# lmxyy/sige

Measured on AMD Instinct MI355X. Metric: DDPM-256 U-Net sparse (SIGE) forwards/s, higher is better.
Workload: dtype f32; 1 GPU; DDPM 256x256 church U-Net (ch128, mult 1-1-2-2-4-4, 113.7M params, random init), 1.2% square edit, one edited image per GPU, hipGraph replay, NHWC activations, in-place scatter ...; batch_per_gpu=1, resolution=256, parallelism=dp1

## Files before the change

### include/sige_hip.h

```cpp
#ifndef SIGE_HIP_H
#define SIGE_HIP_H

#include <stddef.h>
#include <stdint.h>

#ifdef __cplusplus
extern "C" {
#endif

#define SIGE_HIP_VERSION 309

enum {
    SIGE_HIP_OK = 0,
    SIGE_HIP_EINVAL = -1,
    SIGE_HIP_EUNSUPPORTED = -2,
    SIGE_HIP_ELAUNCH = -3,
    SIGE_HIP_ENODEVICE = -4
};

enum { SIGE_HIP_ACT_IDENTITY = 0, SIGE_HIP_ACT_SWISH = 1,
       SIGE_HIP_ACT_RELU = 2, SIGE_HIP_ACT_LEAKY = 3 , SIGE_HIP_ACT_TANH = 4 };

enum {
    SIGE_HIP_TUNE_CONV_TILE_MT = 0,
// ... 343 lines not shown
int sige_hip_conv3x3_small_cin_tiles_nhwc_f32(const float *x, int64_t strideB, int64_t strideC, int64_t strideH, int64_t strideW,
                                              int B, int Cin, int H, int W,
                                              const float *weight, const float *bias, int Cout,
                                              const int32_t *active_indices, int N, int bH, int bW,
                                              float *out, void *stream);

size_t sige_hip_group_norm_affine_workspace(int B, int C, int H, int W, int groups);
int sige_hip_group_norm_affine_f32(const float *x, int B, int C, int H, int W, int groups, float eps,
                                   const float *gamma, const float *beta, float *workspace,
                                   float *scale, float *shift, void *stream);

size_t sige_hip_group_norm_affine_nhwc_workspace(int B, int C, int H, int W, int groups);
int sige_hip_group_norm_affine_nhwc_f32(const float *x, int B, int C, int H, int W, int groups, float eps,
                                        const float *gamma, const float *beta, float *workspace,
                                        float *scale, float *shift, void *stream);

int sige_hip_group_norm_affine_nhwc_bias_f32(const float *x, int B, int C, int H, int W, int groups, float eps,
                                             const float *gamma, const float *beta, const float *channel_bias,
                                             float *workspace, float *scale, float *shift, void *stream);

int sige_hip_group_norm_affine_from_stats_f32(const float *stats1, int tiles1, int C1, int count1,
                                              const float *stats2, int tiles2, int C2, int count2,
                                              int B, int groups, float eps, const float *gamma, const float *beta,
                                              const float *channel_bias, float *scale, float *shift, void *stream);

int sige_hip_channel_stats_tiles(int H, int W);
int sige_hip_channel_stats_nhwc_f32(const float *x, int B, int C, int H, int W, float *stats, void *stream);

size_t sige_hip_attention_workspace(int B, int C, int HW);
int sige_hip_attention_f32(const float *qkv, int B, int C, int HW, float scale, float *workspace,
                           float *out, void *stream);
int sige_hip_attention_nhwc_f32(const float *qkv, int B, int C, int HW, float scale, float *workspace,
                                float *out, void *stream);
size_t sige_hip_attention_fused_workspace(int B, int C, int HW);
int sige_hip_attention_fused_nhwc_f32(const float *qkv, int B, int C, int HW, float scale, float *workspace,
                                      float *out, void *stream);

size_t sige_hip_block_conv_packed_size_f16x3(int Cout, int Cin, int kH, int kW, int R, int S,
                                            int strideH, int strideW, int groups);
int sige_hip_block_conv_pack_f16x3(const float *w, int Cout, int Cin, int kH, int kW,
                                  float *packed, void *stream);
int sige_hip_block_conv_nhwc_f16x3(const float *x, int T, int Cin, int R, int S,
                                  const float *packed, const float *bias, int Cout, int kH, int kW,
                                  int strideH, int strideW, float *out, void *stream);
int sige_hip_block_conv_nhwc_keyed(int compute, const float *x, const int32_t *count_key, int B, int N, int Cin, int R, int S,
                                   const float *packed, const float *bias, int Cout, int kH, int kW,
                                   int strideH, int strideW, float *out, void *stream);
int sige_hip_gather_conv_nhwc_f16x3(const float *x, const float *x2, int B, int C1, int C2, int H, int W,
                                   int bH, int bW, const int32_t *active_indices, int N,
                                   const float *scale, int scaleB, int scaleC,
                                   const float *shift, int shiftB, int shiftC,
                                   int activation,
                                   const float *packed, const float *bias, int Cout, int kH, int kW,
                                   int strideH, int strideW,
                                   int to_full, int offsetH, int offsetW, const float *residual, int Ho, int Wo,
                                   float *workspace, size_t workspace_floats,
                                   const float *out_scale, const float *out_shift, int out_activation,
                                   int upsample2x,
                                   float *twin0, const float *twin0_scale, const float *twin0_shift,
                                   float *twin1, const float *twin1_scale, const float *twin1_shift,
                                   float *out, void *stream);
int sige_hip_scatter_gather_conv_nhwc_f16x3(const float *x, const float *y, int B, int Cin, int H, int W,
                                           int Rx, int Sx, int bH, int bW,
                                           const int32_t *active_indices, int N, const int32_t *scatter_map,
                                           const float *scale, int scaleB, int scaleC,
                                           const float *shift, int shiftB, int shiftC,
// ... 106 lines not shown
```

### sige_amd/build.py

```python
import os
import subprocess
import sys

PKG = os.path.dirname(os.path.abspath(__file__))
REPO = os.path.dirname(PKG)
CSRC = os.path.join(PKG, "csrc")
LIB_DIR = os.path.join(PKG, "lib")
LIB = os.path.join(LIB_DIR, "libsige_hip.so")
SOURCES = ["api.hip", "plan.hip", "gather.hip", "scatter.hip", "reduce_mask.hip", "mask_pipeline.hip", "block_conv.hip", "conv_k3s1.hip", "conv_k1.hip",
           "conv_k3s2.hip", "conv_k3s1_nhwc.hip", "conv_k1_nhwc.hip", "conv_k3s2_nhwc.hip", "conv_k3s1_nhwc_w8.hip", "conv_k1_nhwc_w8.hip", "conv_k3s1_nhwc_h.hip", "conv_k1_nhwc_h.hip", "conv_k3s1_nhwc_x.hip", "conv_k1_nhwc_x.hip", "conv_k3s1_nhwc_c16.hip", "conv_k3s1_nhwc_h_c16.hip", "conv_k3s1_nhwc_x_c16.hip", "conv_pair_nhwc_x_t4.hip", "conv_pair_nhwc_x_f4.hip",
           "conv_pair_nhwc_t4.hip", "conv_pair_nhwc_t8.hip", "conv_pair_nhwc_f4.hip", "conv_pair_nhwc_f8.hip", "conv_pair_nhwc_h_t4.hip", "conv_pair_nhwc_h_f4.hip", "conv_wide.hip", "conv_wide_k3_p8.hip", "conv_wide_k3_f32.hip", "conv_wide_k1_p8.hip", "conv_wide_pair_f32.hip", "conv_wide_pair_x3.hip", "conv_wide_pair_f16.hip", "group_norm.hip", "attention.hip", "attention_fused.hip", "attention_tokens.hip", "nhwc_ops.hip", "conv_out.hip", "conv_in.hip", "spade_ops.hip", "conv_tile3.hip", "conv_tile3_f32.hip", "token_ops.hip", "conv_tile3_f16.hip"]
FLAGS = ["--offload-arch=gfx950", "-O3", "-std=c++17", "-fPIC", "-ffp-contract=off", "-Wno-unused-result"]


def source_hash() -> str:
    import hashlib

    h = hashlib.sha256(" ".join(FLAGS).encode())
    for f in sorted(os.listdir(CSRC)):
        if f.endswith((".hip", ".hpp", ".h")):
            h.update(f.encode())
            h.update(open(os.path.join(CSRC, f), "rb").read())
    h.update(open(os.path.join(REPO, "include", "sige_hip.h"), "rb").read())
    return h.hexdigest()[:16]
# ... 19 lines not shown
        return True
    t = os.path.getmtime(obj)
    return any(os.path.getmtime(d) > t for d in [src, *headers])


TUNING_UNITS = ("api.hip", "block_conv.hip", "gather.hip", "conv_wide.hip", "attention_tokens.hip", "conv_out.hip", "conv_tile3.hip")
TUNING_LIB = os.path.join(LIB_DIR, "libsige_hip_tuning.so")


def _compile_cmd(src: str, obj: str, defs=()):
    return [_hipcc(), *FLAGS, "-DSIGE_TU_ID=%d" % SOURCES.index(src), *defs, "-I" + os.path.join(REPO, "include"), "-I" + CSRC, "-c",
            os.path.join(CSRC, src), "-o", obj]


def _headers():
    headers = [os.path.join(CSRC, f) for f in os.listdir(CSRC) if f.endswith((".hpp", ".h"))]
    headers.append(os.path.join(REPO, "include", "sige_hip.h"))
    return headers


def _headers_of(src: str, headers):
    return (headers if src.startswith("conv_wide") else [h for h in headers if not h.endswith("conv_wide.hpp")] if src.startswith(("conv_k", "conv_pair", "conv_tile3", "block_conv"))
            else [h for h in headers if not h.endswith(("conv_mfma.hpp", "conv_wide.hpp", "conv_tile3.hpp"))])


def _run_all(procs):
    for cmd, p in procs:
        if p.wait() != 0:
            raise RuntimeError("hipcc failed: " + " ".join(cmd))


def build_tuning(force: bool = False, verbose: bool = True) -> str:
    build(force=force, verbose=verbose)
    tdir = os.path.join(LIB_DIR, "tuning")
    os.makedirs(tdir, exist_ok=True)
    headers = _headers()
    objs, procs = [], []
    for src in SOURCES:
        if src in TUNING_UNITS:
            obj = os.path.join(tdir, src.replace(".hip", ".o"))
            if force or _stale(obj, os.path.join(CSRC, src), _headers_of(src, headers)):
                cmd = _compile_cmd(src, obj, ["-DSIGE_HIP_TUNING"])
                if verbose:
                    print(" ".join(cmd), flush=True)
                procs.append((cmd, subprocess.Popen(cmd)))
        else:
            obj = os.path.join(LIB_DIR, src.replace(".hip", ".o"))
        objs.append(obj)
    _run_all(procs)
    if procs or not os.path.isfile(TUNING_LIB) or os.path.getmtime(TUNING_LIB) < os.path.getmtime(LIB):
        subprocess.check_call([_hipcc(), "--offload-arch=gfx950", "-shared", "-fPIC", *objs, "-o", TUNING_LIB])
    return TUNING_LIB


def build_probe(verbose: bool = True) -> str:
    build_tuning(verbose=verbose)
    tag = os.environ.get("SIGE_PROBE_TAG", "")
    only = os.environ.get("SIGE_PROBE_ONLY", "").split()
    pdir = os.path.join(LIB_DIR, "probe" + tag)
    os.makedirs(pdir, exist_ok=True)
    objs, procs = [], []
    wide = bool(os.environ.get("SIGE_PROBE_WIDE"))
    for src in SOURCES:
        if (src.startswith("conv_wide") if wide else
                src.startswith(("conv_k", "conv_pair", "conv_tile3", "block_conv")) and (not only or src in only or src.startswith("block_conv"))):
            obj = os.path.join(pdir, src.replace(".hip", ".o"))
# ... 51 lines not shown
```

### sige_amd/csrc/nhwc_ops.hip

```cpp
#include "common.hpp"

namespace sige {

constexpr int kT = 256;

__device__ __forceinline__ float4 ld4(const float *p) { return *reinterpret_cast<const float4 *>(p); }
__device__ __forceinline__ void st4(float *p, float4 v) { *reinterpret_cast<float4 *>(p) = v; }
__device__ __forceinline__ void st4_out(float *p, float4 v) { store_out4(p, v); }
typedef _Float16 h16x4 __attribute__((ext_vector_type(4)));
__device__ __forceinline__ float4 ld4(const _Float16 *p) {
    const h16x4 h = *reinterpret_cast<const h16x4 *>(p);
    return make_float4((float)h[0], (float)h[1], (float)h[2], (float)h[3]);
}
__device__ __forceinline__ void st4(_Float16 *p, float4 v) {
    const h16x4 h = {(_Float16)v.x, (_Float16)v.y, (_Float16)v.z, (_Float16)v.w};
    *reinterpret_cast<h16x4 *>(p) = h;
}

template <int ACT>
__device__ __forceinline__ float4 affine_act4(float4 z, const float *scale, const float *shift, int so, int c) {
    if (scale) { const float4 s = ld4(scale + so + c); z.x = s.x * z.x; z.y = s.y * z.y; z.z = s.z * z.z; z.w = s.w * z.w; }
    if (shift) { const float4 s = ld4(shift + so + c); z.x = s.x + z.x; z.y = s.y + z.y; z.z = s.z + z.z; z.w = s.w + z.w; }
    z.x = activate<ACT>(z.x); z.y = activate<ACT>(z.y); z.z = activate<ACT>(z.z); z.w = activate<ACT>(z.w);
    return z;
// ... 196 lines not shown
    const int b = blockIdx.z;
    const int i0 = blockIdx.y * 16, j0 = blockIdx.x * 16;
    const int tid = threadIdx.x, wave = tid >> 6, lane = tid & 63;
    const int kq = lane >> 4, n = lane & 15;
    const int C3 = 3 * C, cw = C / 4;
    const float *qa = qkv + ((size_t)b * HW + i0 + n) * C3 + wave * cw + kq * 4;
    const float *kb = qkv + ((size_t)b * HW + j0 + n) * C3 + C + wave * cw + kq * 4;
    f32x4 acc0 = {0.f, 0.f, 0.f, 0.f}, acc1 = {0.f, 0.f, 0.f, 0.f};
    for (int s0 = 0; s0 < cw; s0 += 128) {
        float4 a4[8], b4[8];
#pragma unroll
        for (int u = 0; u < 8; ++u) {
            const int s = s0 + 16 * u;
            const bool ok = s < cw;
            a4[u] = ok ? ld4(qa + s) : make_float4(0.f, 0.f, 0.f, 0.f);
            b4[u] = ok ? ld4(kb + s) : make_float4(0.f, 0.f, 0.f, 0.f);
        }
#pragma unroll
        for (int u = 0; u < 8; ++u) {
            acc0 = __builtin_amdgcn_mfma_f32_16x16x4f32(a4[u].x, b4[u].x, acc0, 0, 0, 0);
            acc1 = __builtin_amdgcn_mfma_f32_16x16x4f32(a4[u].y, b4[u].y, acc1, 0, 0, 0);
            acc0 = __builtin_amdgcn_mfma_f32_16x16x4f32(a4[u].z, b4[u].z, acc0, 0, 0, 0);
            acc1 = __builtin_amdgcn_mfma_f32_16x16x4f32(a4[u].w, b4[u].w, acc1, 0, 0, 0);
        }
    }
#pragma unroll
    for (int r = 0; r < 4; ++r) red[wave][4 * kq + r][n] = acc0[r] + acc1[r];
    __syncthreads();
    const int qi = tid >> 4, kj = tid & 15;
    const float v = (red[0][qi][kj] + red[1][qi][kj]) + (red[2][qi][kj] + red[3][qi][kj]);
    S[((size_t)b * HW + i0 + qi) * HW + j0 + kj] = v * scale;
}

__global__ __launch_bounds__(kT) void attn_apply_nhwc_kernel(const float *__restrict__ qkv, const float *__restrict__ S,
                                                            int C, int HW, float *__restrict__ out) {
    extern __shared__ __attribute__((aligned(16))) float P[];
    const int PS = HW + 4;
    const int b = blockIdx.z;
    const int i0 = blockIdx.y * 16, c0 = blockIdx.x * 64;
    const int tid = threadIdx.x, wave = tid >> 6, lane = tid & 63;
    const int kq = lane >> 4, n = lane & 15;
    const int c = c0 + wave * 16 + n;
    const bool cok = c < C;
    const size_t rs = (size_t)3 * C;
    const __amdgpu_buffer_rsrc_t r_v = __builtin_amdgcn_make_buffer_rsrc(
        const_cast<float *>(qkv + (size_t)b * HW * 3 * C + 2 * C), 0,
        (unsigned)min((size_t)0x7fffffff, ((size_t)HW * 3 * C - 2 * C) * sizeof(float)), 0x00020000);
    const int v_lane = ((cok ? c : 0) + kq * (int)rs) * (int)sizeof(float);
    const int v_step = 4 * (int)rs * (int)sizeof(float);
    float bv[64];
    auto load_values = [&](int j0) {
        const int nk = min(256, HW - j0) / 4;
#pragma unroll
        for (int u = 0; u < 64; ++u)
            bv[u] = __builtin_bit_cast(float, __builtin_amdgcn_raw_buffer_load_b32(r_v, v_lane, (j0 / 4 + min(u, nk - 1)) * v_step, 0));
    };
    {
        const int row = tid >> 4, l16 = tid & 15;
        const float *srow = S + ((size_t)b * HW + i0 + row) * HW;
        if (HW <= 256) {
            float4 t[4];
#pragma unroll
            for (int u = 0; u < 4; ++u) {
                const int j = l16 * 4 + 64 * u;
                const float4 q4 = ld4(srow + min(j, HW - 4));
                t[u] = j < HW ? q4 : make_float4(-INFINITY, -INFINITY, -INFINITY, -INFINITY);
            }
            load_values(0);
            float m = -INFINITY;
#pragma unroll
            for (int u = 0; u < 4; ++u) m = fmaxf(fmaxf(m, fmaxf(t[u].x, t[u].y)), fmaxf(t[u].z, t[u].w));
            m = row16_max(m);
            float sum = 0.f;
#pragma unroll
            for (int u = 0; u < 4; ++u) {
                if (l16 * 4 + 64 * u < HW) {
                    t[u].x = expf(t[u].x - m); t[u].y = expf(t[u].y - m); t[u].z = expf(t[u].z - m); t[u].w = expf(t[u].w - m);
                    sum += (t[u].x + t[u].y) + (t[u].z + t[u].w);
                }
            }
            sum = row16_sum(sum);
            const float inv = 1.0f / sum;
#pragma unroll
            for (int u = 0; u < 4; ++u) {
                const int j = l16 * 4 + 64 * u;
                if (j < HW) {
                    t[u].x *= inv; t[u].y *= inv; t[u].z *= inv; t[u].w *= inv;
                    st4(P + row * PS + j, t[u]);
                }
            }
        } else {
            load_values(0);
            float m = -INFINITY;
            for (int j = l16 * 4; j < HW; j += 64) {
                const float4 t = ld4(srow + j);
                st4(P + row * PS + j, t);
                m = fmaxf(fmaxf(m, fmaxf(t.x, t.y)), fmaxf(t.z, t.w));
            }
#pragma unroll
            for (int o = 8; o > 0; o >>= 1) m = fmaxf(m, __shfl_xor(m, o, 16));
            float sum = 0.f;
            for (int j = l16 * 4; j < HW; j += 64) {
                float4 t = ld4(P + row * PS + j);
                t.x = expf(t.x - m); t.y = expf(t.y - m); t.z = expf(t.z - m); t.w = expf(t.w - m);
                sum += (t.x + t.y) + (t.z + t.w);
                st4(P + row * PS + j, t);
            }
#pragma unroll
            for (int o = 8; o > 0; o >>= 1) sum += __shfl_xor(sum, o, 16);
            const float inv = 1.0f / sum;
            for (int j = l16 * 4; j < HW; j += 64) {
                float4 t = ld4(P + row * PS + j);
                t.x *= inv; t.y *= inv; t.z *= inv; t.w *= inv;
                st4(P + row * PS + j, t);
            }
        }
    }
    __syncthreads();
    const float *pa = P + n * PS + kq;
    f32x4 acc0 = {0.f, 0.f, 0.f, 0.f}, acc1 = {0.f, 0.f, 0.f, 0.f};
    for (int j0 = 0; j0 < HW; j0 += 256) {
        const int nk = min(256, HW - j0) / 4;
        if (j0 > 0) load_values(j0);
#pragma unroll
        for (int u = 0; u < 64; ++u) {
            const float av = pa[j0 + 4 * min(u, nk - 1)];
            const float bb = u < nk ? bv[u] : 0.f;
            if (u & 1) acc1 = __builtin_amdgcn_mfma_f32_16x16x4f32(av, bb, acc1, 0, 0, 0);
            else acc0 = __builtin_amdgcn_mfma_f32_16x16x4f32(av, bb, acc0, 0, 0, 0);
        }
    }
    if (cok) {
#pragma unroll
        for (int r = 0; r < 4; ++r) out[((size_t)b * HW + i0 + 4 * kq + r) * C + c] = acc0[r] + acc1[r];
    }
}

}

using namespace sige;

static bool al16(const void *p) { return (reinterpret_cast<uintptr_t>(p) & 15) == 0; }

static bool affine_shape(const float *scale, int sB, int sC, const float *shift, int tB, int tC, int B, int C, int *aff_sb) {
    *aff_sb = 0;
    for (int k = 0; k < 2; ++k) {
        const float *p = k ? shift : scale;
        const int pb = k ? tB : sB, pc = k ? tC : sC;
        if (!p) continue;
        if (!((pb == 1 || pb == B) && pc == C) || !al16(p)) return false;
        if (pb > 1) *aff_sb = C;
    }
    if (scale && shift && sB != tB) return false;
    return true;
}

template <typename XT>
static int gather_nhwc_impl(const XT *x, int B, int C, int H, int W, int bH, int bW,
                            const int32_t *active_indices, int N,
                            const float *scale, int scaleB, int scaleC,
                            const float *shift, int shiftB, int shiftC,
                            int activation, float *out, void *stream) {
    if (B < 0 || C <= 0 || H <= 0 || W <= 0 || bH <= 0 || bW <= 0 || N < 0) return SIGE_HIP_EINVAL;
    if (activation != SIGE_HIP_ACT_IDENTITY && activation != SIGE_HIP_ACT_SWISH) return SIGE_HIP_EUNSUPPORTED;
    const int hp_shift = stacked_shift(H);
    if (hp_shift < 0 || (hp_shift && B != 1)) return SIGE_HIP_EUNSUPPORTED;
    if ((long)B * N == 0) return SIGE_HIP_OK;
// ... 248 lines not shown
template <typename ST, typename DT>
__global__ __launch_bounds__(kT) void convert4_kernel(const ST *__restrict__ src, DT *__restrict__ dst, size_t n4) {
    for (size_t u = (size_t)blockIdx.x * kT + threadIdx.x; u < n4; u += (size_t)gridDim.x * kT) st4(dst + u * 4, ld4(src + u * 4));
}

extern "C" int sige_hip_convert_f16_f32(const void *src, float *dst, size_t n, void *stream) {
    SIGE_PLAN_HOOK(sige_hip_convert_f16_f32, src, dst, n, stream);
    if (!src || !dst) return SIGE_HIP_EINVAL;
    if (n == 0) return SIGE_HIP_OK;
    if (n % 4 || (reinterpret_cast<uintptr_t>(src) & 7) || !al16(dst)) return SIGE_HIP_EUNSUPPORTED;
    convert4_kernel<_Float16, float><<<grid_for((long)(n / 4)), kT, 0, as_stream(stream)>>>(static_cast<const _Float16 *>(src), dst, n / 4);
    return launch_status();
}

extern "C" int sige_hip_convert_f32_f16(const float *src, void *dst, size_t n, void *stream) {
    SIGE_PLAN_HOOK(sige_hip_convert_f32_f16, src, dst, n, stream);
    if (!src || !dst) return SIGE_HIP_EINVAL;
    if (n == 0) return SIGE_HIP_OK;
    if (n % 4 || (reinterpret_cast<uintptr_t>(dst) & 7) || !al16(src)) return SIGE_HIP_EUNSUPPORTED;
    convert4_kernel<float, _Float16><<<grid_for((long)(n / 4)), kT, 0, as_stream(stream)>>>(src, static_cast<_Float16 *>(dst), n / 4);
    return launch_status();
}

extern "C" int sige_hip_attention_nhwc_f32(const float *qkv, int B, int C, int HW, float scale, float *workspace,
                                           float *out, void *stream) {
    SIGE_PLAN_HOOK(sige_hip_attention_nhwc_f32, qkv, B, C, HW, scale, workspace, out, stream);
    if (B <= 0 || C <= 0 || HW <= 0) return SIGE_HIP_EINVAL;
    if (!qkv || !workspace || !out) return SIGE_HIP_EINVAL;
    if (HW % 16 || C % 64 || B > 65535 || !al16(qkv) || !al16(workspace)) return SIGE_HIP_EUNSUPPORTED;
    const size_t lds = (size_t)16 * (HW + 4) * sizeof(float);
    if (lds > 64 * 1024 || (size_t)HW * 3 * C * sizeof(float) >= 0x7fffffffu) return SIGE_HIP_EUNSUPPORTED;
    hipStream_t st = as_stream(stream);
    attn_scores_nhwc_kernel<<<dim3(HW / 16, HW / 16, B), kT, 0, st>>>(qkv, C, HW, scale, workspace);
    attn_apply_nhwc_kernel<<<dim3(ceil_div(C, 64), HW / 16, B), kT, lds, st>>>(qkv, workspace, C, HW, out);
    return launch_status(2);
}
```

### sige_amd/hip.py

```python
import ctypes
import os
import threading
from typing import Optional, Tuple

import torch

_PKG = os.path.dirname(os.path.abspath(__file__))
LIB_PATH = os.environ.get("SIGE_HIP_LIB", os.path.join(_PKG, "lib", "libsige_hip.so"))

ACT = {"identity": 0, "swish": 1}
ACT_EXT = {"identity": 0, "relu": 2, "leaky": 3, "tanh": 4}

_c_int, _c_vp, _c_sz = ctypes.c_int, ctypes.c_void_p, ctypes.c_size_t
_lib = None

_BC = [_c_vp, _c_int, _c_int, _c_int, _c_int]

_SIGNATURES = {
    "sige_hip_version": (_c_int, []),
    "sige_hip_error_string": (ctypes.c_char_p, [_c_int]),
    "sige_hip_device_arch": (ctypes.c_char_p, []),
    "sige_hip_launch_count": (ctypes.c_int64, []),
    "sige_hip_last_launch_device": (_c_int, []),
    "sige_hip_preload": (_c_int, []),
# ... 57 lines not shown
    "sige_hip_scatter_gather_conv_nhwc_f16c": (
        _c_int, [_c_vp, _c_vp] + [_c_int] * 8 + [_c_vp, _c_int, _c_vp] + [_c_vp, _c_int, _c_int] * 2 + [_c_int, _c_vp, _c_vp]
        + [_c_int] * 5 + [_c_vp, _c_vp]),
    "sige_hip_scatter_gather_conv_scatter_nhwc_f16c": (
        _c_int, [_c_vp, _c_vp] + [_c_int] * 8 + [_c_vp, _c_int, _c_vp] + [_c_vp, _c_int, _c_int] * 2 + [_c_int, _c_vp, _c_vp]
        + [_c_int] * 3 + [_c_int, _c_int, _c_vp] + [_c_vp, _c_vp] + [_c_int] * 5 + [_c_vp] * 6 + [_c_vp, _c_vp]),
    "sige_hip_scatter_gather_conv_nhwc_f32": (
        _c_int, [_c_vp, _c_vp] + [_c_int] * 8 + [_c_vp, _c_int, _c_vp] + [_c_vp, _c_int, _c_int] * 2 + [_c_int, _c_vp, _c_vp]
        + [_c_int] * 5 + [_c_vp, _c_vp]),
    "sige_hip_scatter_gather_conv_scatter_nhwc_f32": (
        _c_int, [_c_vp, _c_vp] + [_c_int] * 8 + [_c_vp, _c_int, _c_vp] + [_c_vp, _c_int, _c_int] * 2 + [_c_int, _c_vp, _c_vp]
        + [_c_int] * 3 + [_c_int, _c_int, _c_vp] + [_c_vp, _c_vp] + [_c_int] * 5 + [_c_vp] * 6 + [_c_vp, _c_vp]),
    "sige_hip_gather_nhwc_f32": (
        _c_int, [_c_vp] + [_c_int] * 6 + [_c_vp, _c_int] + [_c_vp, _c_int, _c_int] * 2 + [_c_int, _c_vp, _c_vp]),
    "sige_hip_scatter_gather_nhwc_f32": (
        _c_int, [_c_vp, _c_vp] + [_c_int] * 8 + [_c_vp, _c_int, _c_vp] + [_c_vp, _c_int, _c_int] * 2 + [_c_int, _c_vp, _c_vp]),
    "sige_hip_spade_modulate_nhwc_f32": (
        _c_int, [_c_vp, _c_vp, _c_vp, _c_int, _c_int, _c_int] + [_c_vp, _c_int, _c_int] * 2 + [_c_vp, _c_vp, _c_vp, _c_int, _c_int, _c_int]
        + [_c_int] * 6 + [_c_vp, _c_int, _c_int, ctypes.c_float, _c_vp, _c_vp]),
    "sige_hip_scatter_nhwc_f32": (
        _c_int, [_c_vp, _c_vp] + [_c_int] * 10 + [_c_vp, _c_vp, _c_int, _c_int, _c_int, _c_vp, _c_int, _c_vp, _c_vp]),
    "sige_hip_scatter_with_block_residual_nhwc_f32": (
        _c_int, [_c_vp] * 4 + [_c_int] * 12 + [_c_vp, _c_vp, _c_int, _c_int, _c_int] * 2 + [_c_int, _c_vp, _c_vp]),
    "sige_hip_group_norm_affine_nhwc_workspace": (_c_sz, [_c_int] * 5),
    "sige_hip_group_norm_affine_nhwc_f32": (_c_int, [_c_vp] + [_c_int] * 5 + [ctypes.c_float] + [_c_vp] * 6),
    "sige_hip_group_norm_affine_nhwc_bias_f32": (_c_int, [_c_vp] + [_c_int] * 5 + [ctypes.c_float] + [_c_vp] * 7),
    "sige_hip_conv3x3_small_cout_nhwc_f32": (
        _c_int, [_c_vp] + [_c_int] * 4 + [_c_vp, _c_int, _c_int] * 2 + [_c_int, _c_vp, _c_vp, _c_int, _c_vp, _c_vp]),
    "sige_hip_conv3x3_small_cin_nhwc_f32": (
        _c_int, [_c_vp] + [ctypes.c_int64] * 4 + [_c_int] * 4 + [_c_vp, _c_vp, _c_int, _c_vp, _c_vp]),
    "sige_hip_conv3x3_small_cin_tiles_nhwc_f32": (
        _c_int, [_c_vp] + [ctypes.c_int64] * 4 + [_c_int] * 4 + [_c_vp, _c_vp, _c_int, _c_vp, _c_int, _c_int, _c_int, _c_vp, _c_vp]),
    "sige_hip_attention_nhwc_f32": (_c_int, [_c_vp, _c_int, _c_int, _c_int, ctypes.c_float, _c_vp, _c_vp, _c_vp]),
    "sige_hip_attention_fused_workspace": (_c_sz, [_c_int] * 3),
    "sige_hip_attention_fused_nhwc_f32": (_c_int, [_c_vp, _c_int, _c_int, _c_int, ctypes.c_float, _c_vp, _c_vp, _c_vp]),
    "sige_hip_block_conv_packed_size_f16x3": (_c_sz, [_c_int] * 9),
    "sige_hip_block_conv_pack_f16x3": (_c_int, [_c_vp] + [_c_int] * 4 + [_c_vp, _c_vp]),
    "sige_hip_block_conv_nhwc_f16x3": (_c_int, [_c_vp] + [_c_int] * 4 + [_c_vp, _c_vp] + [_c_int] * 5 + [_c_vp, _c_vp]),
    "sige_hip_gather_conv_nhwc_f16x3": (
        _c_int, [_c_vp, _c_vp] + [_c_int] * 7 + [_c_vp, _c_int] + [_c_vp, _c_int, _c_int] * 2 + [_c_int, _c_vp, _c_vp]
        + [_c_int] * 5 + [_c_int, _c_int, _c_int, _c_vp, _c_int, _c_int, _c_vp, _c_sz, _c_vp, _c_vp, _c_int, _c_int] + [_c_vp] * 6
        + [_c_vp, _c_vp]),
    "sige_hip_scatter_gather_conv_nhwc_f16x3": (
        _c_int, [_c_vp, _c_vp] + [_c_int] * 8 + [_c_vp, _c_int, _c_vp] + [_c_vp, _c_int, _c_int] * 2 + [_c_int, _c_vp, _c_vp]
        + [_c_int] * 5 + [_c_vp, _c_vp]),
    "sige_hip_scatter_gather_conv_scatter_nhwc_f16x3": (
        _c_int, [_c_vp, _c_vp] + [_c_int] * 8 + [_c_vp, _c_int, _c_vp] + [_c_vp, _c_int, _c_int] * 2 + [_c_int, _c_vp, _c_vp]
        + [_c_int] * 3 + [_c_int, _c_int, _c_vp] + [_c_vp, _c_vp] + [_c_int] * 5 + [_c_vp] * 6 + [_c_vp, _c_vp]),
    "sige_hip_affine_act_nhwc_f32": (_c_int, [_c_vp] + [_c_int] * 4 + [_c_vp, _c_vp, _c_int, _c_int, _c_vp, _c_vp]),
    "sige_hip_wide_conv_supported": (_c_int, [_c_int] * 5),
    "sige_hip_wide_conv_packed_size": (_c_sz, [_c_int] * 5),
    "sige_hip_wide_conv_pack": (_c_int, [_c_vp] + [_c_int] * 6 + [_c_vp, _c_vp]),
    "sige_hip_wide_conv_workspace": (_c_sz, [_c_int] * 8),
    "sige_hip_wide_conv_nhwc": (
        _c_int, [_c_vp, _c_vp] + [_c_int] * 6 + [_c_vp, _c_vp, _c_int, _c_int] + [_c_vp, _c_int, _c_int, _c_vp, _c_int, _c_int, _c_int]
        + [_c_vp, _c_vp, _c_vp, _c_int] + [_c_vp] * 6 + [_c_vp, _c_sz, _c_vp, _c_vp, _c_vp]),
    "sige_hip_release_graph_tickets": (_c_int, []),
    "sige_hip_channel_stats_tiles": (_c_int, [_c_int, _c_int]),
    "sige_hip_channel_stats_nhwc_f32": (_c_int, [_c_vp] + [_c_int] * 4 + [_c_vp, _c_vp]),
    "sige_hip_group_norm_affine_from_stats_f32": (
        _c_int, [_c_vp, _c_int, _c_int, _c_int, _c_vp, _c_int, _c_int, _c_int, _c_int, _c_int, ctypes.c_float] + [_c_vp] * 6),
    "sige_hip_attention_tokens_supported": (_c_int, [_c_int] * 4),
    "sige_hip_attention_tokens_f32": (_c_int, [_c_vp] * 3 + [_c_int] * 5 + [ctypes.c_float, _c_vp, _c_vp]),
    "sige_hip_gather_nhwc_f16": (
        _c_int, [_c_vp] + [_c_int] * 6 + [_c_vp, _c_int] + [_c_vp, _c_int, _c_int] * 2 + [_c_int, _c_vp, _c_vp]),
    "sige_hip_scatter_gather_nhwc_f16": (
# ... 1644 lines not shown
                                                    _stream(x))
    if status == UNSUPPORTED:
        return None
    _check(status, "affine_act_cl")
    return out


FUSED_ATTENTION = False


def attention_cl(qkv: torch.Tensor, scale: float):
    qkv = _req_cl(qkv, "qkv")
    B, C3, H, W = qkv.shape
    C, HW = C3 // 3, H * W
    out = _empty_cl((B, C, H, W), qkv.device)
    if FUSED_ATTENTION:
        n = int(lib().sige_hip_attention_fused_workspace(B, C, HW))
        if n:
            ws = torch.empty(n, dtype=torch.float32, device=qkv.device)
            status = lib().sige_hip_attention_fused_nhwc_f32(qkv.data_ptr(), B, C, HW, float(scale), ws.data_ptr(), out.data_ptr(),
                                                             _stream(qkv))
            if status != UNSUPPORTED:
                _check(status, "attention_fused_cl")
                return out
    ws = torch.empty(B * HW * HW, dtype=torch.float32, device=qkv.device)
    status = lib().sige_hip_attention_nhwc_f32(qkv.data_ptr(), B, C, HW, float(scale), ws.data_ptr(), out.data_ptr(),
                                               _stream(qkv))
    if status == UNSUPPORTED:
        return None
    _check(status, "attention_cl")
    return out


def attention_tokens(q: torch.Tensor, k: torch.Tensor, v: torch.Tensor, heads: int, scale: float) -> Optional[torch.Tensor]:
    if not (q.is_cuda and q.dtype == k.dtype == v.dtype == torch.float32 and q.dim() == k.dim() == v.dim() == 3):
        return None
    B, Nq, C = q.shape
    if tuple(k.shape) != tuple(v.shape) or k.shape[0] != B or k.shape[2] != C:
        return None
    Nk = k.shape[1]
    if not lib().sige_hip_attention_tokens_supported(Nq, Nk, C, heads):
        return None
    q, k, v = (t if t.is_contiguous() else t.contiguous() for t in (q, k, v))
    out = torch.empty((B, Nq, C), dtype=torch.float32, device=q.device)
    status = lib().sige_hip_attention_tokens_f32(q.data_ptr(), k.data_ptr(), v.data_ptr(), B, Nq, Nk, C, heads, float(scale),
                                                 out.data_ptr(), _stream(q))
    if status == UNSUPPORTED:
        return None
    _check(status, "attention_tokens")
    return out


def conv3x3_small_cout_cl(x, weight, bias, scale=None, shift=None, activationName="identity"):
    x = _req_cl(x, "x")
    B, C, H, W = x.shape
    w = _req(weight.detach(), torch.float32, "weight")
    Cout = w.shape[0]
    if tuple(w.shape[1:]) != (C, 3, 3):
        return None
    bias_keep = _vec(bias, "bias")
    (sa, s_keep), (ta, t_keep) = _cvec(scale, "scale"), _cvec(shift, "shift")
    out = _empty_cl((B, Cout, H, W), x.device)
    status = lib().sige_hip_conv3x3_small_cout_nhwc_f32(x.data_ptr(), B, C, H, W, *sa, *ta, _act(activationName),
                                                        w.data_ptr(), _p(bias_keep), Cout, out.data_ptr(), _stream(x))
    if status == UNSUPPORTED:
        return None
# ... 35 lines not shown
```

### sige_amd/workloads/ddpm_unet.py

```python
import math
from dataclasses import dataclass
from typing import Optional, Tuple

import torch
from torch import nn
from torch.nn import functional as F

from ..nn import Gather, Scatter, ScatterGather, ScatterWithBlockResidual, SIGEConv2d, SIGEModel, SIGEModule, paired_convs
from ..nn.deferred import lazy_cat
from ..nn.dense import fast_full_pass, full_conv2d, fused_conv2d, group_norm_affine, input_conv2d


@dataclass
class DDPMConfig:
    ch: int = 128
    ch_mult: Tuple[int, ...] = (1, 1, 2, 2, 4, 4)
    num_res_blocks: int = 2
    attn_resolutions: Tuple[int, ...] = (16,)
    in_ch: int = 3
    out_ch: int = 3
    resolution: int = 256
    main_block: Optional[int] = 6
    shortcut_block: Optional[int] = 4
    sparse_threshold: int = 64
# ... 7 lines not shown


def timestep_embedding(t: torch.Tensor, dim: int) -> torch.Tensor:
    half = dim // 2
    freq = torch.exp(torch.arange(half, dtype=torch.float32, device=t.device) * (-math.log(10000) / (half - 1)))
    arg = t.float()[:, None] * freq[None, :]
    emb = torch.cat([arg.sin(), arg.cos()], dim=1)
    return F.pad(emb, (0, 1)) if dim % 2 else emb


def norm_affine(x: torch.Tensor, norm: nn.GroupNorm, fast: bool = False, cbias: Optional[torch.Tensor] = None,
                x2: Optional[torch.Tensor] = None):
    if fast and x.is_cuda:
        assert x.shape[0] == 1, "SIGE caches one original image"
        sc, sh = group_norm_affine(x, norm, cbias, x2=x2, make_stats=True)
        return sc.reshape(-1), sh.reshape(-1)
    if x2 is not None:
        x = torch.cat([x, x2], dim=1)
    n, c, h, w = x.shape
    assert n == 1, "SIGE caches one original image"
    if cbias is not None:
        x = x + cbias.reshape(1, -1, 1, 1)
    g = norm.num_groups
    var, mean = torch.var_mean(x.reshape(g, -1), dim=1, unbiased=False)
    inv = torch.rsqrt(var + norm.eps).repeat_interleave(c // g)
    mu = mean.repeat_interleave(c // g)
    scale = inv * norm.weight
    shift = norm.bias - mu * scale
    return scale, shift


def _as4(v: torch.Tensor) -> torch.Tensor:
    return v.reshape(1, -1, 1, 1)


class _TwinProducer:

    def _twin_scatter(self):
        return None

    def _twins_ok(self) -> bool:
        return True

    def register_twin(self, key, scale: torch.Tensor, shift: torch.Tensor) -> bool:
        if not self._twins_ok():
            return False
        sct = self._twin_scatter()
        if sct is not None:
            return sct.twins.register(key, scale, shift)
        from ..nn.scatter import twin_key_cache_id, twins_for

        regs = self.__dict__.setdefault("twin_regs", {})
        if key not in regs and len(twins_for(regs, twin_key_cache_id(key))) >= 2:
            return False
        regs[key] = (scale, shift)
        return True

    def unregister_twin(self, key):
        sct = self._twin_scatter()
        if sct is not None:
            sct.twins.unregister(key)
        self.__dict__.setdefault("twin_regs", {}).pop(key, None)

    def _my_twins(self) -> dict:
        from ..nn.scatter import twins_for

# ... 218 lines not shown
                else:
                    h = fused_conv2d(self.conv1, x, s1, t1, "swish", x2=x2, out_affine=(s2, t2, "swish"))
            join()
            return self._produced(fused_conv2d(self.conv2, h, residual=skip, twins=self._my_twins()))
        if self.cin == self.cout:
            skip = x if x2 is None else torch.cat([x, x2], dim=1)
        else:
            skip, join = self._shortcut_async(lambda: fused_conv2d(self.nin_shortcut, x, x2=x2), x)
        join()
        h = fused_conv2d(self.conv1, x, s1, t1, "swish", x2=x2)
        return fused_conv2d(self.conv2, h, s2, t2, "swish", residual=skip)


class AttnBlock(SIGEModule, _TwinProducer):
    def __init__(self, cfg: DDPMConfig, ch: int, sparse: bool):
        super().__init__()
        self.ch = ch
        self.edit_batch = 1
        self.twin_regs = {}
        self.quirk = cfg.reference_attn_quirk
        self.sparse = sparse and cfg.shortcut_block is not None
        Conv = SIGEConv2d if self.sparse else nn.Conv2d
        self.norm = nn.GroupNorm(cfg.groups, ch, eps=cfg.eps)
        self.qkv = Conv(ch, 3 * ch, 1, 1, 0)
        self.proj_out = Conv(ch, ch, 1, 1, 0)
        if self.sparse:
            self.gather1 = Gather(self.qkv, cfg.shortcut_block)
            self.scatter1 = Scatter(self.gather1)
            self.gather2 = Gather(self.proj_out, cfg.shortcut_block)
            self.scatter2 = Scatter(self.gather2)
        self.affine = {}
        self.plain = False

    def clear_cache(self):
        self.affine = {}

    def forward(self, x: torch.Tensor) -> torch.Tensor:
        if self.mode == "full" and self.plain:
            h = self.norm(x)
        elif self.mode == "full":
            h = self.gather1(x) if self.sparse else x
            s, t = norm_affine(h, self.norm, fast_full_pass(self.qkv))
            self.affine[self.cache_id] = (_as4(s).contiguous(), _as4(t).contiguous())
            if not self.sparse:
                qkv = full_conv2d(self.qkv, h, _as4(s), _as4(t), "identity")
                return full_conv2d(self.proj_out, self._attention(qkv), residual=x)
            h = h * _as4(s) + _as4(t)
        else:
            s, t = self.affine[self.cache_id]
            if self.quirk:
                s, t = s[:, :1].expand_as(s).contiguous(), t[:, :1].expand_as(t).contiguous()
            if not self.sparse and self.mode == "sparse":
                return self._dense_sparse(x, s, t)
            h = self.gather1(x, s, t) if self.sparse else x * s + t
        plain = self.mode == "full" and self.plain
        qkv = self.qkv(h)
        if self.sparse and not plain:
            qkv = self.scatter1(qkv)
        b, _, hh, ww = qkv.shape
        q, k, v = qkv.reshape(b, 3, self.ch, hh * ww).unbind(1)
        attn = torch.softmax(torch.bmm(q.transpose(1, 2), k) * (self.ch ** -0.5), dim=2)
        h = torch.bmm(v, attn.transpose(1, 2)).reshape(b, self.ch, hh, ww)
        if self.sparse and not plain:
            h = self.gather2(h)
        h = self.proj_out(h)
        return self.scatter2(h, x) if (self.sparse and not plain) else h + x


    def _attention(self, qkv):
        if self.edit_batch > 1 and qkv.shape[0] == 1:
            from ..stacked import tall, untall

            return tall(self._attention(untall(qkv, self.edit_batch)))
        b, _, hh, ww = qkv.shape
        if qkv.is_cuda and qkv.dtype == torch.float32:
            from .. import hip

            if hip.is_cl(qkv):
                out = hip.attention_cl(qkv, self.ch ** -0.5)
                if out is not None:
                    return out
            if hip.attention_supported(self.ch, hh * ww):
                return hip.attention(qkv, self.ch ** -0.5)
        q, k, v = qkv.reshape(b, 3, self.ch, hh * ww).unbind(1)
        attn = torch.softmax(torch.bmm(q.transpose(1, 2), k) * (self.ch ** -0.5), dim=2)
        return torch.bmm(v, attn.transpose(1, 2)).reshape(b, self.ch, hh, ww)

    def _twins_ok(self) -> bool:
        return not self.sparse

    def _dense_sparse(self, x, s, t):
        qkv = fused_conv2d(self.qkv, x, s, t, "identity")
        return self._produced(fused_conv2d(self.proj_out, self._attention(qkv), residual=x, twins=self._my_twins()))


class Upsample(SIGEModule, _TwinProducer):

    def _twin_scatter(self):
        return self.scatter

    def __init__(self, cfg: DDPMConfig, ch: int):
        super().__init__()
        self.conv = SIGEConv2d(ch, ch, 3, 1, 1)
        self.gather = Gather(self.conv, cfg.main_block)
        self.scatter = Scatter(self.gather)
        self.plain = False

    def forward(self, x):
        if self.mode == "sparse" and self.gather.fuses_upsample(x):
            return self._produced(self.scatter.forward_fused(self.conv, self.gather(x, upsample2x=True)))
        if self.mode == "full" and not self.plain and x.is_cuda:
            from ..nn import dense as _dense

            if _dense.fast_full_pass(self.conv):
                self.gather.note_full_input((2 * x.shape[2], 2 * x.shape[3]))
                return self.scatter(full_conv2d(self.conv, x, upsample2x=True, stats=True))
        x = F.interpolate(x, scale_factor=2.0, mode="nearest")
        if self.mode == "sparse":
            return self._produced(self.scatter.forward_fused(self.conv, self.gather(x)))
        if self.plain and self.mode == "full":
            return self.conv(x)
        return self.scatter(self.conv(self.gather(x)))


# ... 183 lines not shown
```

Baseline: 747.4 forward/s.

## Fold attention output projection into V weights and fuse residual epilogue

Precomputes W_proj·W_v, so the qkv conv emits already-projected values and the separate proj_out 1x1 conv disappears. Projection bias, residual add and twin swish outputs move into the attention-apply kernel epilogue. This removes one conv launch and a full activation round trip per attention block, at the cost of a weight fold cached on parameter versions and small numeric differences from reassociation. The build script also skips rebuilding the tuning library when it is up to date.

```diff
diff --git a/include/sige_hip.h b/include/sige_hip.h
--- a/include/sige_hip.h
+++ b/include/sige_hip.h
@@ -399,6 +399,11 @@
                            float *out, void *stream);
 int sige_hip_attention_nhwc_f32(const float *qkv, int B, int C, int HW, float scale, float *workspace,
                                 float *out, void *stream);
+int sige_hip_attention_residual_nhwc_f32(const float *qkv, int B, int C, int HW, float scale, float *workspace,
+                                         const float *bias, const float *residual,
+                                         float *twin0, const float *twin0_scale, const float *twin0_shift,
+                                         float *twin1, const float *twin1_scale, const float *twin1_shift,
+                                         float *out, void *stream);
 size_t sige_hip_attention_fused_workspace(int B, int C, int HW);
 int sige_hip_attention_fused_nhwc_f32(const float *qkv, int B, int C, int HW, float scale, float *workspace,
                                       float *out, void *stream);
diff --git a/sige_amd/build.py b/sige_amd/build.py
--- a/sige_amd/build.py
+++ b/sige_amd/build.py
@@ -75,6 +75,11 @@
 
 def build_tuning(force: bool = False, verbose: bool = True) -> str:
     build(force=force, verbose=verbose)
+    if not force and os.path.isfile(TUNING_LIB):
+        t = os.path.getmtime(TUNING_LIB)
+        deps = [os.path.join(CSRC, f) for f in os.listdir(CSRC)] + [os.path.join(REPO, "include", "sige_hip.h"), LIB]
+        if all(os.path.getmtime(d) <= t for d in deps):
+            return TUNING_LIB
     tdir = os.path.join(LIB_DIR, "tuning")
     os.makedirs(tdir, exist_ok=True)
     headers = _headers()
diff --git a/sige_amd/csrc/nhwc_ops.hip b/sige_amd/csrc/nhwc_ops.hip
--- a/sige_amd/csrc/nhwc_ops.hip
+++ b/sige_amd/csrc/nhwc_ops.hip
@@ -252,8 +252,15 @@
     S[((size_t)b * HW + i0 + qi) * HW + j0 + kj] = v * scale;
 }
 
+struct AttnEpilogue {
+    const float *bias, *residual;
+    float *twin0, *twin1;
+    const float *tscale0, *tshift0, *tscale1, *tshift1;
+};
+
+template <bool EPI>
 __global__ __launch_bounds__(kT) void attn_apply_nhwc_kernel(const float *__restrict__ qkv, const float *__restrict__ S,
-                                                            int C, int HW, float *__restrict__ out) {
+                                                            int C, int HW, float *__restrict__ out, AttnEpilogue e) {
     extern __shared__ __attribute__((aligned(16))) float P[];
     const int PS = HW + 4;
     const int b = blockIdx.z;
@@ -268,6 +275,18 @@
         (unsigned)min((size_t)0x7fffffff, ((size_t)HW * 3 * C - 2 * C) * sizeof(float)), 0x00020000);
     const int v_lane = ((cok ? c : 0) + kq * (int)rs) * (int)sizeof(float);
     const int v_step = 4 * (int)rs * (int)sizeof(float);
+    float e_bias = 0.f, e_s0 = 0.f, e_t0 = 0.f, e_s1 = 0.f, e_t1 = 0.f, e_res[4] = {0.f, 0.f, 0.f, 0.f};
+    auto load_epilogue = [&]() {
+        if constexpr (EPI) {
+            const int cc = cok ? c : 0;
+            e_bias = (e.bias ? e.bias : qkv)[cc];
+            e_s0 = (e.twin0 ? e.tscale0 : qkv)[cc]; e_t0 = (e.twin0 ? e.tshift0 : qkv)[cc];
+            e_s1 = (e.twin1 ? e.tscale1 : qkv)[cc]; e_t1 = (e.twin1 ? e.tshift1 : qkv)[cc];
+            const float *rp = (e.residual ? e.residual : qkv) + ((size_t)b * HW + i0 + 4 * kq) * C + cc;
+#pragma unroll
+            for (int r = 0; r < 4; ++r) e_res[r] = rp[(size_t)r * C];
+        }
+    };
     float bv[64];
     auto load_values = [&](int j0) {
         const int nk = min(256, HW - j0) / 4;
@@ -286,6 +305,7 @@
                 const float4 q4 = ld4(srow + min(j, HW - 4));
                 t[u] = j < HW ? q4 : make_float4(-INFINITY, -INFINITY, -INFINITY, -INFINITY);
             }
+            load_epilogue();
             load_values(0);
             float m = -INFINITY;
 #pragma unroll
@@ -310,6 +330,7 @@
                 }
             }
         } else {
+            load_epilogue();
             load_values(0);
             float m = -INFINITY;
             for (int j = l16 * 4; j < HW; j += 64) {
@@ -352,7 +373,17 @@
     }
     if (cok) {
 #pragma unroll
-        for (int r = 0; r < 4; ++r) out[((size_t)b * HW + i0 + 4 * kq + r) * C + c] = acc0[r] + acc1[r];
+        for (int r = 0; r < 4; ++r) {
+            const size_t at = ((size_t)b * HW + i0 + 4 * kq + r) * C + c;
+            float s = acc0[r] + acc1[r];
+            if constexpr (EPI) {
+                if (e.bias) s += e_bias;
+                if (e.residual) s += e_res[r];
+                if (e.twin0) { float t = e_s0 * s; t = e_t0 + t; e.twin0[at] = swish(t); }
+                if (e.twin1) { float t = e_s1 * s; t = e_t1 + t; e.twin1[at] = swish(t); }
+            }
+            out[at] = s;
+        }
     }
 }
 
@@ -667,6 +698,31 @@
     if (lds > 64 * 1024 || (size_t)HW * 3 * C * sizeof(float) >= 0x7fffffffu) return SIGE_HIP_EUNSUPPORTED;
     hipStream_t st = as_stream(stream);
     attn_scores_nhwc_kernel<<<dim3(HW / 16, HW / 16, B), kT, 0, st>>>(qkv, C, HW, scale, workspace);
-    attn_apply_nhwc_kernel<<<dim3(ceil_div(C, 64), HW / 16, B), kT, lds, st>>>(qkv, workspace, C, HW, out);
+    attn_apply_nhwc_kernel<false><<<dim3(ceil_div(C, 64), HW / 16, B), kT, lds, st>>>(qkv, workspace, C, HW, out, AttnEpilogue{});
     return launch_status(2);
 }
+
+extern "C" int sige_hip_attention_residual_nhwc_f32(const float *qkv, int B, int C, int HW, float scale, float *workspace,
+                                                    const float *bias, const float *residual,
+                                                    float *twin0, const float *twin0_scale, const float *twin0_shift,
+                                                    float *twin1, const float *twin1_scale, const float *twin1_shift,
+                                                    float *out, void *stream) {
+    SIGE_PLAN_HOOK(sige_hip_attention_residual_nhwc_f32, qkv, B, C, HW, scale, workspace, bias, residual, twin0, twin0_scale, twin0_shift, twin1, twin1_scale, twin1_shift, out, stream);
+    if (B <= 0 || C <= 0 || HW <= 0) return SIGE_HIP_EINVAL;
+    if (!qkv || !workspace || !out) return SIGE_HIP_EINVAL;
+    if ((twin0 && !(twin0_scale && twin0_shift)) || (twin1 && !(twin1_scale && twin1_shift))) return SIGE_HIP_EINVAL;
+    if (!al16(bias) || !al16(residual) || !al16(twin0) || !al16(twin0_scale) || !al16(twin0_shift) || !al16(twin1) ||
+        !al16(twin1_scale) || !al16(twin1_shift))
+        return SIGE_HIP_EINVAL;
+    if (HW % 16 || C % 64 || B > 65535 || !al16(qkv) || !al16(workspace)) return SIGE_HIP_EUNSUPPORTED;
+    const size_t lds = (size_t)16 * (HW + 4) * sizeof(float);
+    if (lds > 64 * 1024 || (size_t)HW * 3 * C * sizeof(float) >= 0x7fffffffu) return SIGE_HIP_EUNSUPPORTED;
+    AttnEpilogue e{};
+    e.bias = bias; e.residual = residual;
+    e.twin0 = twin0; e.tscale0 = twin0_scale; e.tshift0 = twin0_shift;
+    e.twin1 = twin1; e.tscale1 = twin1_scale; e.tshift1 = twin1_shift;
+    hipStream_t st = as_stream(stream);
+    attn_scores_nhwc_kernel<<<dim3(HW / 16, HW / 16, B), kT, 0, st>>>(qkv, C, HW, scale, workspace);
+    attn_apply_nhwc_kernel<true><<<dim3(ceil_div(C, 64), HW / 16, B), kT, lds, st>>>(qkv, workspace, C, HW, out, e);
+    return launch_status(2);
+}
diff --git a/sige_amd/hip.py b/sige_amd/hip.py
--- a/sige_amd/hip.py
+++ b/sige_amd/hip.py
@@ -113,6 +113,7 @@
     "sige_hip_conv3x3_small_cin_tiles_nhwc_f32": (
         _c_int, [_c_vp] + [ctypes.c_int64] * 4 + [_c_int] * 4 + [_c_vp, _c_vp, _c_int, _c_vp, _c_int, _c_int, _c_int, _c_vp, _c_vp]),
     "sige_hip_attention_nhwc_f32": (_c_int, [_c_vp, _c_int, _c_int, _c_int, ctypes.c_float, _c_vp, _c_vp, _c_vp]),
+    "sige_hip_attention_residual_nhwc_f32": (_c_int, [_c_vp, _c_int, _c_int, _c_int, ctypes.c_float, _c_vp] + [_c_vp] * 10),
     "sige_hip_attention_fused_workspace": (_c_sz, [_c_int] * 3),
     "sige_hip_attention_fused_nhwc_f32": (_c_int, [_c_vp, _c_int, _c_int, _c_int, ctypes.c_float, _c_vp, _c_vp, _c_vp]),
     "sige_hip_block_conv_packed_size_f16x3": (_c_sz, [_c_int] * 9),
@@ -1823,6 +1824,30 @@
     return out
 
 
+def attention_residual_cl(qkv: torch.Tensor, scale: float, bias: Optional[torch.Tensor] = None,
+                          residual: Optional[torch.Tensor] = None, twins: Optional[dict] = None):
+    qkv = _req_cl(qkv, "qkv")
+    B, C3, H, W = qkv.shape
+    C, HW = C3 // 3, H * W
+    out = _empty_cl((B, C, H, W), qkv.device)
+    bias_keep = _vec(bias, "bias")
+    if bias_keep is not None and bias_keep.numel() != C:
+        raise RuntimeError("attention_residual_cl: bias needs one entry per channel")
+    if residual is not None:
+        residual = _req_cl(residual, "residual")
+        if tuple(residual.shape) != tuple(out.shape):
+            raise RuntimeError("attention_residual_cl: residual must be shaped like the output")
+    tw = [(key, _empty_cl((B, C, H, W), qkv.device), sc, sh) for key, (sc, sh) in list((twins or {}).items())[:2]]
+    targs, twin_keep = _twin_args([(b, sc, sh) for _, b, sc, sh in tw] or None, out, C, "attention_residual_cl")
+    ws = torch.empty(B * HW * HW, dtype=torch.float32, device=qkv.device)
+    status = lib().sige_hip_attention_residual_nhwc_f32(qkv.data_ptr(), B, C, HW, float(scale), ws.data_ptr(), _p(bias_keep),
+                                                        _p(residual), *targs, out.data_ptr(), _stream(qkv))
+    if status == UNSUPPORTED:
+        return None
+    _check(status, "attention_residual_cl")
+    return out, {key: b for key, b, _, _ in tw}
+
+
 def attention_tokens(q: torch.Tensor, k: torch.Tensor, v: torch.Tensor, heads: int, scale: float) -> Optional[torch.Tensor]:
     if not (q.is_cuda and q.dtype == k.dtype == v.dtype == torch.float32 and q.dim() == k.dim() == v.dim() == 3):
         return None
diff --git a/sige_amd/workloads/ddpm_unet.py b/sige_amd/workloads/ddpm_unet.py
--- a/sige_amd/workloads/ddpm_unet.py
+++ b/sige_amd/workloads/ddpm_unet.py
@@ -63,6 +63,22 @@
 
 def _as4(v: torch.Tensor) -> torch.Tensor:
     return v.reshape(1, -1, 1, 1)
+
+
+FOLD_ATTN_PROJ = True
+
+
+def fold_proj_into_qkv(w_qkv: torch.Tensor, b_qkv: Optional[torch.Tensor], w_p: torch.Tensor, b_p: Optional[torch.Tensor]):
+    C = w_p.shape[0]
+    wq = w_qkv.detach().reshape(3 * C, C)
+    wp = w_p.detach().reshape(C, C).double()
+    bq = torch.zeros(3 * C, dtype=wq.dtype, device=wq.device) if b_qkv is None else b_qkv.detach()
+    w = torch.cat([wq[:2 * C], (wp @ wq[2 * C:].double()).to(wq.dtype)]).reshape(3 * C, C, 1, 1)
+    b = torch.cat([bq[:2 * C], torch.zeros_like(bq[2 * C:])])
+    bp = wp @ bq[2 * C:].double()
+    if b_p is not None:
+        bp = bp + b_p.detach().double()
+    return w.contiguous(), b, bp.to(wq.dtype)
 
 
 class _TwinProducer:
@@ -347,9 +363,6 @@
         self.affine = {}
         self.plain = False
 
-    def clear_cache(self):
-        self.affine = {}
-
     def forward(self, x: torch.Tensor) -> torch.Tensor:
         if self.mode == "full" and self.plain:
             h = self.norm(x)
@@ -404,7 +417,54 @@
     def _twins_ok(self) -> bool:
         return not self.sparse
 
+    def clear_cache(self):
+        self.affine = {}
+        self.__dict__.pop("_fold", None)
+
+    def folded_proj(self):
+        params = (self.qkv.weight, self.qkv.bias, self.proj_out.weight, self.proj_out.bias)
+        key = tuple(None if p is None else (p.data_ptr(), p._version, tuple(p.shape), p.device, p.dtype) for p in params)
+        key += (getattr(self.qkv, "compute_dtype", "f32"),)
+        entry = self.__dict__.get("_fold")
+        if entry is None or entry[0] != key:
+            w, b, bp = fold_proj_into_qkv(*params)
+            conv = nn.Conv2d(self.ch, 3 * self.ch, 1, 1, 0, device="meta")
+            conv.weight, conv.bias = nn.Parameter(w, requires_grad=False), nn.Parameter(b, requires_grad=False)
+            conv.compute_dtype = key[-1]
+            entry = (key, conv, bp)
+            self.__dict__["_fold"] = entry
+        return entry[1], entry[2]
+
+    def _fold_ok(self, x) -> bool:
+        if not (FOLD_ATTN_PROJ and x.is_cuda and x.dtype == torch.float32):
+            return False
+        if getattr(self.qkv, "compute_dtype", "f32") != "f32" or getattr(self.proj_out, "compute_dtype", "f32") != "f32":
+            return False
+        from .. import hip
+
+        return hip.is_cl(x) and not hip.FUSED_ATTENTION
+
     def _dense_sparse(self, x, s, t):
+        refused = self.__dict__.setdefault("_fold_refused", set())
+        if tuple(x.shape) not in refused and self._fold_ok(x):
+            from .. import hip
+
+            conv, bp = self.folded_proj()
+            qkv = fused_conv2d(conv, x, s, t, "identity")
+            if hip.is_cl(qkv):
+                E = self.edit_batch if qkv.shape[0] == 1 else 1
+                if E > 1:
+                    from ..stacked import tall, untall
+
+                    res = hip.attention_residual_cl(untall(qkv, E), self.ch ** -0.5, bp, residual=untall(x, E), twins=self._my_twins())
+                    if res is not None:
+                        res = (tall(res[0]), {k: tall(v) for k, v in res[1].items()})
+                else:
+                    res = hip.attention_residual_cl(qkv, self.ch ** -0.5, bp, residual=x, twins=self._my_twins())
+                if res is not None:
+                    res[0]._sige_twins = res[1]
+                    return self._produced(res[0])
+            refused.add(tuple(x.shape))
         qkv = fused_conv2d(self.qkv, x, s, t, "identity")
         return self._produced(fused_conv2d(self.proj_out, self._attention(qkv), residual=x, twins=self._my_twins()))
 
```

Result: faster. 771.5 forward/s, median of 6 (+3.2%).
